# lRomul/sensorium

Measured on AMD Instinct MI355X. Metric: training clips/sec/GPU (DwiseNeuro fwd+bwd, B=32 T=32 36x64) at 1/2/4/8 GPUs, higher is better.
Workload: dtype bf16

## Files before the change

sensorium_amd/csrc/dwn_api.hip:

```cpp
#include "dwn_internal.h"
#include "dwn_kernels.h"
#include <string.h>
#include <math.h>

static thread_local char g_err[512] = "";
#ifndef DWN_EVAL_CHAIN
#define DWN_EVAL_CHAIN 1
#endif

extern "C" size_t dwn_dw_spatial_rc_blob_bytes(int E, int Cin);
extern "C" int dwn_dw_spatial_rc_supported(int dtype, int Cin, int E, int ks, int stride, int Hin, int Win);
extern "C" int dwn_dw_spatial_rc_prep(const float* w_pw, const float* w_dws, const float* bn1_coef, int E, int Cin, void* blob,
                                      int device, void* stream);
extern "C" int dwn_dw_spatial_fwd_rc(const dwn_dw_spatial_rc_fwd_args* a, int device, void* stream);
bool dw_spatial_bwd_rc_supported(const DwSpatialBwd& a, int dtype);
bool dw_spatial_fwd_rc_walk_supported(const DwSpatialFwd& a, int dtype);

int dwn_set_error(int code, const char* msg) {
    snprintf(g_err, sizeof(g_err), "dwn error %d: %s", code, msg ? msg : "");
    return code;
}

#define TRY(x) do { int rc__ = (x); if (rc__ != 0) return rc__; } while (0)

// ... 124 lines not shown
GemmTN tn_base(const LoadDesc& p, int pk, const LoadDesc& q, int qk, int M, int R, int Cc, float* dw, i64 lddw, int groups) {
    GemmTN g; memset(&g, 0, sizeof(g));
    g.p = p; g.p_kind = pk; g.q = q; g.q_kind = qk; g.M = M; g.R = R; g.Cc = Cc; g.dw = dw; g.lddw = lddw;
    g.groups = groups; g.nsplit = 0;
    return g;
}

struct BlockWs {
    void *wpw, *wpwl;
    float *wdws, *wdwt;
    double *st1, *st2, *st3, *st4, *stsc;
    long long* pooled;
    float *abc1, *abc2, *abc3, *abc4, *abcsc, *ident3;
    float *dgp, *dhp, *dps;
    void* bp; float* r3; float* gacc;
    float* tacc;
    void* wgated;
    void* rcblob;
    double* gram;
    float* pb;
    char* zero_beg; char* zero_end;
    size_t bytes;
};
#ifndef PWL_GATED_MIN_ROWS
#define PWL_GATED_MIN_ROWS 8192
#endif
static bool pwl_gated_weights(const dwn_block_args& a) {
    const int bk = a.dtype == DWN_BF16 ? 64 : 32;
    return ((a.T * a.Hout * a.Wout) % 128) == 0 && a.Cmid > bk && (a.dtype != DWN_BF16 || a.T * a.Hout * a.Wout >= PWL_GATED_MIN_ROWS);
}
// ... 44 lines not shown
    if (!backward && block_y1_free(a)) w.gram = c.take<double>((size_t)(a.Cin + 8) * a.Cin);
    size_t z1 = c.off;
    if (backward) {
        w.abc1 = c.take<float>(3 * (size_t)a.Cmid);
        w.abc2 = c.take<float>(3 * (size_t)a.Cmid);
        w.abc3 = c.take<float>(3 * (size_t)a.Cmid);
        w.abc4 = c.take<float>(3 * (size_t)a.Cout);
        w.abcsc = c.take<float>(3 * (size_t)a.Cout);
        w.ident3 = c.take<float>(3 * (size_t)a.Cmid);
        w.dgp = c.take<float>((size_t)a.B * a.Cmid);
        w.dhp = c.take<float>((size_t)a.B * a.se_r);
        w.dps = c.take<float>((size_t)a.B * a.Cmid);
        w.bp = c.take<char>((size_t)a.Cin * (a.Cmid + a.Cin) * ts);
        w.gacc = c.take<float>(pw_fold_floats(a.Cin));
        w.r3 = w.gacc + (size_t)a.Cin * a.Cin;
        w.tacc = c.take<float>(pw_wgrad_tacc_floats(a.Cmid, a.Cin));
        if (pwl_bwd_per_sample(a)) w.pb = c.take<float>((size_t)a.B * a.Cout * a.Cmid);
    }
    w.bytes = c.off + 256;
    if (base) { w.zero_beg = (char*)base + z0; w.zero_end = (char*)base + z1; }
    return w;
}

static inline int f32_split_of(int policy, bool eval_forward) {
    return policy == DWN_F32_SPLIT3 ? 1 : policy == DWN_F32_NATIVE ? 0 : (eval_forward ? 1 : 0);
}

ResGeom geom_of(const dwn_block_args& a) {
    ResGeom gm;
    gm.BT = a.B * a.T; gm.T = a.T; gm.Hin = a.Hin; gm.Win = a.Win; gm.Hout = a.Hout; gm.Wout = a.Wout;
// ... 343 lines not shown
        g.stats = tr ? w.st4 : nullptr; g.stat_nchan = a.Cout; g.f32_split = f32_split_of(a.f32_products, !tr);
        PROF(DWN_FAM_PWL_FWD, launch_gemm_nn(g, dt, s));
    }
    ResGeom gm = geom_of(a);
    if (bs) {
        if (!(y1_free && identity_sc)) PROF(DWN_FAM_RESID_FWD, k_shortcut_stats(xin, gm, w.stsc, dt, s));
        TRY(k_bn_finalize_train(fin_job(w.st4, a.Cout, (double)Mout, a.bn4, a.Cout),
                                 fin_job(w.stsc, a.Cin, (double)Mout, a.bnsc, a.Cout), a.momentum, a.eps, s));
    }
    PROF(DWN_FAM_RESID_FWD, k_residual_fwd(xin, a.y4, a.bn4.coef, a.bnsc.coef, a.drop_scale, gm, a.out_pe_t, a.out_pe_h,
                                           a.out_pe_w, a.out, dt, s));
    return 0;
}

static int pw_backward(int dt, const void* dh1, const void* a0, const float* w_pw, const float* abc, int E, int Cin, i64 M,
                       void* bp, float* gacc, float* r3, float* tacc, void* da0, float* dw, const void* res,
                       const float* res_abc, int res_C, const ResGeom* rg, hipStream_t s) {
    const int res_n = res ? res_C / Cin : 0;
    const bool gathered = res && rg && rg->hinv;
    if (res && (!res_abc || res_C % Cin || res_n < 1 || res_n > 2))
        return dwn_set_error(-2, "pw_backward: the shortcut term needs res_abc and res_C in {Cin, 2 Cin}");
    if (res && !pw_bwd_fused_supported(dt, M, E, Cin))
        return dwn_set_error(-3, "pw_backward: the shortcut term is built into the one-pass kernel only (dwn_pw_bwd_fused_supported)");
    TRY(k_pw_bwd_prep(w_pw, abc, E, Cin, bp, gacc, r3, dt, (res && !gathered) ? res_abc : nullptr, res_C, s));
    if (pw_bwd_fused_supported(dt, M, E, Cin)) {
        PROF(DWN_FAM_PW_DGRAD, launch_pw_bwd_fused(dh1, a0, bp, r3, da0, tacc, M, E, Cin, dt, res, res_abc, res_n,
                                                   gathered ? rg->hinv : nullptr, gathered ? rg->winv : nullptr, gathered ? rg->Hin : 0,
                                                   gathered ? rg->Win : 0, gathered ? rg->Hout : 0, gathered ? rg->Wout : 0, s));
    } else {
        {
            GemmNN g = nn_base(ld_plain(dh1, E), LD_PLAIN, bp, (i64)E + Cin, da0, Cin, (int)M, Cin, E + Cin, 1);
            g.epi = EPI_STORE_CAT; g.a2 = a0; g.a2_ld = Cin; g.K1 = E; g.bias = r3;
            PROF(DWN_FAM_PW_DGRAD, launch_gemm_nn(g, dt, s));
        }
        {
            LoadDesc cat = ld_plain(dh1, E);
            cat.q = a0; cat.ld2 = Cin; cat.cat_c1 = E; cat.cat_c2 = Cin;
            GemmTN g = tn_base(cat, LD_CAT1, ld_plain(a0, Cin), LD_PLAIN, (int)M, E + Cin + 8, Cin, tacc, Cin, 1);
            PROF(DWN_FAM_PW_WGRAD, launch_gemm_tn(g, dt, s));
// ... 19 lines not shown
    float* dg = reinterpret_cast<float*>(w.pooled);
    const bool y1_free = block_y1_free(a);
    {
        PrepArgs pa;
        bool ok = pa.zero(w.zero_beg, ((size_t)(w.zero_end - w.zero_beg) + 15) & ~(size_t)15);
        ok = ok && pa.packw(a.w_pwl, w.wpwl, 1, a.Cout, a.Cmid, 1, a.Cmid, a.Cout);
        if (y1_free) ok = ok && pa.packw(a.w_pw, w.wpw, 1, a.Cmid, a.Cin, 0, a.Cmid, a.Cin);
        ok = ok && pa.packdw(a.w_dws, w.wdws, a.Cmid, a.ks * a.ks);
        ok = ok && pa.packdw(a.w_dwt, w.wdwt, a.Cmid, a.kt);
        ok = ok && pa.fill(w.ident3, 1.0f, a.Cmid);
        ok = ok && pa.fill(w.ident3 + a.Cmid, 0.0f, 2 * a.Cmid);
        ok = ok && pa.zero(a.dw_dws, (size_t)a.Cmid * a.ks * a.ks * sizeof(float));
        ok = ok && pa.zero(a.dw_dwt, (size_t)a.Cmid * a.kt * sizeof(float));
        ok = ok && pa.zero(a.dw_pwl, (size_t)a.Cout * a.Cmid * sizeof(float));
        if (w.pb) ok = ok && pa.zero(w.pb, (size_t)a.B * a.Cout * a.Cmid * sizeof(float));
        ok = ok && pa.zero(w.gacc, pw_fold_floats(a.Cin) * sizeof(float));
        ok = ok && pa.zero(w.tacc, pw_wgrad_tacc_floats(a.Cmid, a.Cin) * sizeof(float));
        if (!ok) return dwn_set_error(-2, "block_backward: workspace arena and dw_* buffers must be 16-byte aligned");
        TRY(k_prep(pa, dt, s));
    }

    LoadDesc xin = ld_plain(a.x_has_pe ? a.x : a.a0, a.Cin);
    ResGeom gm = geom_of(a);
    PROF(DWN_FAM_RESID_BWD, k_residual_bwd_reduce(xin, a.y4, a.dout, a.bn4.coef, a.bnsc.coef, a.drop_scale, gm, w.st4, w.stsc, dt, s));
    TRY(k_bn_bwd_finalize(bwd_job(w.st4, (double)Mout, a.bn4, w.abc4, a.Cout, frozen),
                          bwd_job(w.stsc, (double)Mout, a.bnsc, w.abcsc, a.Cout, frozen), s));
    PROF(DWN_FAM_RESID_BWD, k_residual_bwd_dy4(a.y4, a.dout, w.abc4, a.drop_scale, gm, a.dy4, dt, s));
    void* du = a.buf_a;
    if (w.pb) {
        {
            GemmTN g = tn_base(ld_plain(a.dy4, a.Cout), LD_PLAIN, ld_plain(a.z3, a.Cmid), LD_PLAIN, (int)Mout, a.Cout,
// ... 43 lines not shown
    TRY(k_bn_bwd_finalize(bwd_job(w.st2, (double)Mout, a.bn2, w.abc2, a.Cmid, frozen), BnBwdJob{}, s));
    void* dh1 = a.buf_a;
    {
        DwSpatialBwd d; memset(&d, 0, sizeof(d));
        d.dy = ld_affine2(a.buf_b, a.y2, a.Cmid, w.abc2, a.Cmid);
        d.y1 = ld_ycoef(y1_free ? nullptr : a.y1, a.Cmid, a.bn1.coef, a.Cmid);
        if (y1_free) { d.a0 = xin.p; d.a0_ld = a.Cin; d.w1 = w.wpw; d.Cin = a.Cin; }
        d.w = w.wdws; d.dh1 = dh1; d.dw = a.dw_dws; d.planes = a.B * a.T; d.Hin = a.Hin; d.Win = a.Win;
        d.Hout = a.Hout; d.Wout = a.Wout; d.C = a.Cmid; d.stride = a.stride; d.ks = a.ks; d.stats = w.st1;
        PROF(DWN_FAM_DWS_BWD, launch_dw_spatial_bwd(d, dt, s));
    }
    TRY(k_bn_bwd_finalize(bwd_job(w.st1, (double)Min, a.bn1, w.abc1, a.Cmid, frozen), BnBwdJob{}, s));
    const bool identity_sc = a.stride == 1 && a.Hin == a.Hout && a.Win == a.Wout;
    const bool dx_folded = a.Cout % a.Cin == 0 && a.Cout / a.Cin <= 2 && dwn_pw_bwd_fused_supported(dt, Min, a.Cmid, a.Cin) &&
                           (identity_sc || (gm.hinv && gm.winv && a.Hin + a.Win <= 512));
    TRY(pw_backward(dt, dh1, xin.p, a.w_pw, w.abc1, a.Cmid, a.Cin, Min, w.bp, w.gacc, w.r3, w.tacc, dx_folded ? a.dx : a.da0, a.dw_pw,
                    dx_folded ? a.dout : nullptr, w.abcsc, a.Cout, (dx_folded && !identity_sc) ? &gm : nullptr, s));
    if (dx_folded) return 0;
    PROF(DWN_FAM_RESID_BWD, k_residual_bwd_dx(xin, a.da0, a.dout, w.abcsc, gm, a.dx, dt, s));
    return 0;
}

int dwn_block_forward_writes(const dwn_block_args* ap) {
    const dwn_block_args& a = *ap;
    if (a.training) return block_y1_free(a) ? 2 : 3;
    if (block_fwd_rc(a)) return 0;
    if (DWN_EVAL_CHAIN && a.dtype == DWN_BF16) {
        DwSpatialFwd f; memset(&f, 0, sizeof(f));
        f.planes = a.B * a.T; f.Hin = a.Hin; f.Win = a.Win; f.Hout = a.Hout; f.Wout = a.Wout; f.C = a.Cmid; f.stride = a.stride; f.ks = a.ks;
        f.in.ld = a.Cmid; f.a0_ld = a.Cin; f.Cin = a.Cin;
        if (dw_spatial_fwd_rc_walk_supported(f, a.dtype)) return 0;
// ... 258 lines not shown
    g_err[0] = 0;
    if (ntensors < 0) return dwn_set_error(-2, "adamw_ema_multi_guarded: ntensors < 0");
    if (max_blocks < 1 || max_blocks > 65535 || ntensors > 65535)
        return dwn_set_error(-2, "adamw_ema_multi_guarded: max_blocks and ntensors are grid dimensions (1 <= max_blocks, both <= 65535)");
    if (!list && ntensors > 0) return dwn_set_error(-1, "adamw_ema_multi_guarded: null table");
    if (!guard) return dwn_set_error(-1, "adamw_ema_multi_guarded: null guard");
    ENTER(device);
    return k_adamw_ema_guarded(list, ntensors, max_blocks, lr, beta1, beta2, eps, weight_decay, ema_decay, grad_scale, guard,
                               (hipStream_t)stream);
}

int dwn_pw_bwd_fused_supported(int dtype, long long M, int E, int Cin) {
    return pw_bwd_fused_supported(dtype, M, E, Cin) ? 1 : 0;
}
size_t dwn_pw_backward_workspace_bytes(int E, int Cin, int dtype) {
    return (size_t)Cin * (E + Cin) * tsize(dtype) + 256 + (pw_fold_floats(Cin) + pw_wgrad_tacc_floats(E, Cin)) * sizeof(float) + 256;
}
int dwn_pw_backward(const dwn_pw_bwd_args* a, int dtype, int device, void* stream) {
    ENTER(device);
    if (!a || !a->dh1 || !a->a0 || !a->w_pw || !a->abc || !a->da0 || !a->dw || !a->ws)
        return dwn_set_error(-1, "pw_backward: null pointer");
    if (a->E <= 0 || a->Cin <= 0 || a->E % 8 || a->Cin % 8 || a->M <= 0 || a->M > 0x7fffffffLL)
        return dwn_set_error(-2, "pw_backward: E and Cin must be positive multiples of 8, 0 < M < 2^31");
    if (a->ws_bytes < dwn_pw_backward_workspace_bytes(a->E, a->Cin, dtype)) return dwn_set_error(-6, "pw_backward: workspace too small");
    hipStream_t s = (hipStream_t)stream;
    Carver c(a->ws, a->ws_bytes);
    void* bp = c.take<char>((size_t)a->Cin * (a->E + a->Cin) * tsize(dtype));
    const size_t nz = pw_fold_floats(a->Cin) + pw_wgrad_tacc_floats(a->E, a->Cin);
    float* gacc = c.take<float>(nz);
    float* r3 = gacc + (size_t)a->Cin * a->Cin;
    float* tacc = gacc + pw_fold_floats(a->Cin);
    TRY(k_zero(gacc, nz * sizeof(float), s));
    ResGeom rg; memset(&rg, 0, sizeof(rg));
    rg.hinv = a->res_hinv; rg.winv = a->res_winv; rg.Hin = a->res_Hin; rg.Win = a->res_Win; rg.Hout = a->res_Hout; rg.Wout = a->res_Wout;
    return pw_backward(dtype, a->dh1, a->a0, a->w_pw, a->abc, a->E, a->Cin, a->M, bp, gacc, r3, tacc, a->da0, a->dw, a->res,
                       a->res_abc, a->res_C, a->res_hinv ? &rg : nullptr, s);
}

int dwn_assemble_inputs(const dwn_clip_desc* descs, int B, int T, int H0, int W0, int H, int W, float pad_fill,
                        float* x, int device, void* stream) {
    ENTER(device);
    if (!descs || !x) return dwn_set_error(-1, "assemble_inputs: null pointer");
    if (B <= 0 || T <= 0 || H0 <= 0 || W0 <= 0) return dwn_set_error(-2, "assemble_inputs: B, T, H0, W0 must be positive");
    if (H < H0 || W < W0) return dwn_set_error(-2, "assemble_inputs: output frame smaller than the video");
    return k_assemble_inputs(descs, B, T, H0, W0, H, W, pad_fill, x, (hipStream_t)stream);
}

int dwn_assemble_targets(const dwn_clip_desc* descs, int B, int T, float* const* targets, const int* n_neurons,
                         int n_mice, int max_neurons, float* mice_weights, int device, void* stream) {
    ENTER(device);
// ... 80 lines not shown
```

sensorium_amd/csrc/dwn_elementwise.hip:

```cpp
#include "dwn_internal.h"
#include "dwn_kernels.h"
#include "dwn_launch.h"

#define NCV 8
#define DISPATCH_T(dtype, CALL_BF, CALL_F) do { if ((dtype) == DWN_BF16) { CALL_BF; } else { CALL_F; } } while (0)

#define SLICE_SETUP(Cval)                                   \
    constexpr int KC = TT<T>::KC;                           \
    const int tid = threadIdx.x;                            \
    const int cv = tid % NCV, pl = tid / NCV;               \
    const int c0 = blockIdx.y * NCV * KC;                   \
    const int chan = c0 + cv * KC;                          \
    const bool chan_ok = chan < (Cval);                     \
    (void)pl; (void)chan_ok;

template <int KC>
__device__ __forceinline__ void slice_stats_flush(float* lstat, const float* s0, const float* s1, int cv,
                                                 int c0, int C, double* stats, int rep) {
    static_assert(NCV == 8, "wave pre-reduction below assumes 8 channel vectors per slice");
    const int tid = threadIdx.x;
    DET_WAVES_BEGIN
#pragma unroll
    for (int i = 0; i < KC; ++i) {
        float a = s0[i], b = s1[i];
// ... 1223 lines not shown
    const int c_end = (part + 1) * per < C ? (part + 1) * per : C;
    for (int c = part * per + tid; c < c_end; c += 256) {
        float acc = 0.f;
        for (int r = 0; r < R; ++r) acc = fmaf(wr[(i64)r * C + c], dhp[r], acc);
        dps[(i64)b * C + c] = acc * inv_s;
    }
}

#define SE_RT 64
__device__ __forceinline__ float wave_sum(float v) {
#pragma unroll
    for (int o = 32; o > 0; o >>= 1) v += __shfl_xor(v, o);
    return v;
}

template <int RP>
__global__ __launch_bounds__(256) void se_mlp_fwd_rows_kernel(const long long* pooled_sum, float inv_s, const float* wr,
                                                              const float* br, const float* we, const float* be, int C,
                                                              int R, float* pmean, float* hid_pre, float* gate,
                                                              const float* __restrict__ w2, void* __restrict__ wg, int N2, int wg_bf16) {
    constexpr int RPW = RP / 4;
    __shared__ float hid[RP];
    __shared__ float gl[256];
    const int b = blockIdx.x, tid = threadIdx.x, lane = tid & 63, wave = tid >> 6;
    const int split = gridDim.y, part = blockIdx.y;
    const int C4 = C >> 2;
    float acc[RPW];
#pragma unroll
    for (int q = 0; q < RPW; ++q) acc[q] = 0.f;
    const longlong2* ps2 = reinterpret_cast<const longlong2*>(pooled_sum + (i64)b * C);
    float4* pm4 = reinterpret_cast<float4*>(pmean + (i64)b * C);
    for (int c4 = lane; c4 < C4; c4 += 64) {
        const longlong2 p0 = ps2[2 * c4], p1 = ps2[2 * c4 + 1];
        float4 v;
        v.x = pool_unfix(p0.x) * inv_s; v.y = pool_unfix(p0.y) * inv_s; v.z = pool_unfix(p1.x) * inv_s; v.w = pool_unfix(p1.y) * inv_s;
        if (part == 0 && wave == 0) pm4[c4] = v;
        float4 w[RPW];
#pragma unroll
        for (int q = 0; q < RPW; ++q) {
            const int r = wave + 4 * q;
            w[q] = reinterpret_cast<const float4*>(wr + (i64)(r < R ? r : R - 1) * C)[c4];
        }
#pragma unroll
        for (int q = 0; q < RPW; ++q)
            acc[q] = fmaf(w[q].x, v.x, fmaf(w[q].y, v.y, fmaf(w[q].z, v.z, fmaf(w[q].w, v.w, acc[q]))));
    }
#pragma unroll
    for (int q = 0; q < RPW; ++q) {
        const float t = wave_sum(acc[q]);
        const int r = wave + 4 * q;
        if (lane == 0 && r < R) {
            const float h = t + br[r];
            if (part == 0) hid_pre[(i64)b * R + r] = h;
            hid[r] = siluf_(h);
        }
    }
    __syncthreads();
    const int per = (C + split - 1) / split;
    const int c_end = (part + 1) * per < C ? (part + 1) * per : C;
    for (int c = part * per + tid; c < c_end; c += 256) {
        float a = be[c];
        const float* wrow = we + (i64)c * R;
#pragma unroll 1
        for (int r0 = 0; r0 < RP; r0 += 16) {
            if (r0 >= R) break;
            float wv[16];
            if ((R & 3) == 0) {
                const float4* w4 = reinterpret_cast<const float4*>(wrow);
                const int nq = R >> 2;
#pragma unroll
                for (int q = 0; q < 4; ++q) {
                    const int qi = (r0 >> 2) + q;
                    const float4 t = w4[qi < nq ? qi : nq - 1];
                    wv[4 * q] = t.x; wv[4 * q + 1] = t.y; wv[4 * q + 2] = t.z; wv[4 * q + 3] = t.w;
                }
            } else {
#pragma unroll
                for (int r = 0; r < 16; ++r) wv[r] = wrow[r0 + r < R ? r0 + r : R - 1];
            }
#pragma unroll
            for (int r = 0; r < 16; ++r) a = fmaf(wv[r], r0 + r < R ? hid[r0 + r] : 0.f, a);
        }
        const float gv = sigmoidf_(a);
        gate[(i64)b * C + c] = gv;
        if (w2 && c - part * per < 256) gl[c - part * per] = gv;
    }
    if (w2) {
        __syncthreads();
        const int c0 = part * per, nc = c_end - c0;
        if (nc > 0) {
            const int tot = N2 * nc;
            for (int i = tid; i < tot; i += 256) {
                const int n = i / nc, cc = i - n * nc;
                const float v = w2[(i64)n * C + c0 + cc] * gl[cc];
                const i64 o = ((i64)b * N2 + n) * C + c0 + cc;
                if (wg_bf16) reinterpret_cast<bf16_t*>(wg)[o] = f2bf(v);
                else reinterpret_cast<float*>(wg)[o] = v;
            }
        }
    }
}

template <int N, int LIVE, int D> struct WaveFold {
    static __device__ __forceinline__ void run(float (&v)[N], int lane) {
        if constexpr (D > 0) {
            if constexpr (LIVE > D) {
                constexpr int H = LIVE / 2;
// ... 81 lines not shown
            float wv[16];
#pragma unroll
            for (int r = 0; r < 16; ++r) wv[r] = wr[(i64)(r0 + r < R ? r0 + r : R - 1) * C + c];
#pragma unroll
            for (int r = 0; r < 16; ++r) a = fmaf(wv[r], r0 + r < R ? dhp[r0 + r] : 0.f, a);
        }
        dps[(i64)b * C + c] = a * inv_s;
    }
}

__global__ __launch_bounds__(256) void se_mlp_wgrad_kernel(const float* dgp, const float* dhp, const float* pmean,
                                                           const float* hid_pre, int B, int C, int R, float* dwr,
                                                           float* dbr, float* dwe, float* dbe) {
    const int c = blockIdx.x * 256 + threadIdx.x;
    const int r = blockIdx.y;
    if (c < C) {
        float a = 0.f, a2 = 0.f, sb = 0.f;
#pragma unroll 8
        for (int b = 0; b < B; ++b) {
            float g = dgp[(i64)b * C + c];
            a = fmaf(g, siluf_(hid_pre[(i64)b * R + r]), a);
            a2 = fmaf(dhp[(i64)b * R + r], pmean[(i64)b * C + c], a2);
            sb += g;
        }
        dwe[(i64)c * R + r] = a;
        dwr[(i64)r * C + c] = a2;
        if (r == 0) dbe[c] = sb;
    }
    if (blockIdx.x == 0 && threadIdx.x == 0) {
        float sb = 0.f;
        for (int b = 0; b < B; ++b) sb += dhp[(i64)b * R + r];
        dbr[r] = sb;
    }
}

int k_se_mlp_fwd(const long long* pooled_sum, float inv_s, const float* wr, const float* br, const float* we,
                 const float* be, int B, int C, int R, float* pmean, float* hid_pre, float* gate, const float* w2, void* wg, int N2,
                 int dtype, int* folded, hipStream_t s) {
    if (folded) *folded = 0;
    if ((C & 3) == 0 && R <= SE_RT && !(((size_t)pooled_sum | (size_t)wr | (size_t)pmean) & 15)) {
        const bool fold = w2 && wg && (C + 7) / 8 <= 256;
        const float* w2f = fold ? w2 : nullptr;
        const int bf = dtype == DWN_BF16 ? 1 : 0;
        if (R <= 16)
            hipLaunchKernelGGL(se_mlp_fwd_rows_kernel<16>, dim3(B, 8), dim3(256), 0, s, pooled_sum, inv_s, wr, br, we, be, C, R,
                               pmean, hid_pre, gate, w2f, wg, N2, bf);
        else if (R <= 32)
            hipLaunchKernelGGL(se_mlp_fwd_rows_kernel<32>, dim3(B, 8), dim3(256), 0, s, pooled_sum, inv_s, wr, br, we, be, C, R,
                               pmean, hid_pre, gate, w2f, wg, N2, bf);
        else
            hipLaunchKernelGGL(se_mlp_fwd_rows_kernel<SE_RT>, dim3(B, 8), dim3(256), 0, s, pooled_sum, inv_s, wr, br, we, be, C,
                               R, pmean, hid_pre, gate, w2f, wg, N2, bf);
        if (folded && fold) *folded = 1;
    } else {
        hipLaunchKernelGGL(se_mlp_fwd_kernel, dim3(B, 8), dim3(256), (C + R) * sizeof(float), s, pooled_sum, inv_s, wr, br,
                           we, be, C, R, pmean, hid_pre, gate);
    }
    DWN_CHECK_LAUNCH();
    return 0;
}
int k_se_mlp_bwd(const float* dg, const float* gate, const float* hid_pre, const float* pmean, const float* wr,
                 const float* we, int B, int C, int R, float inv_s, float* dgp, float* dhp, float* dps, float* dwr,
                 float* dbr, float* dwe, float* dbe, hipStream_t s) {
    if ((R & 1) == 0 && R <= SE_RT && !((size_t)we & 15)) {
#define SE_BWD_FOLD(RP_) do { \
        if ((R & 3) == 0) hipLaunchKernelGGL((se_mlp_bwd_fold_kernel<RP_, 4>), dim3(B, 8), dim3(256), 0, s, dg, gate, hid_pre, wr, we, C, R, inv_s, dgp, dhp, dps); \
        else hipLaunchKernelGGL((se_mlp_bwd_fold_kernel<RP_, 2>), dim3(B, 8), dim3(256), 0, s, dg, gate, hid_pre, wr, we, C, R, inv_s, dgp, dhp, dps); } while (0)
// ... 990 lines not shown
int k_prep(const PrepArgs& pa, int dtype, hipStream_t s) {
    int total = 0;
    for (int i = 0; i < pa.nops; ++i) total += pa.op[i].nblocks;
    if (total == 0) return 0;
    DISPATCH_T(dtype,
        hipLaunchKernelGGL((prep_kernel<bf16_t>), dim3(total), dim3(256), 0, s, pa),
        hipLaunchKernelGGL((prep_kernel<float>), dim3(total), dim3(256), 0, s, pa));
    DWN_CHECK_LAUNCH();
    return 0;
}



template <typename T>
__global__ __launch_bounds__(256) void pw_bwd_prep_kernel(const float* w1, const float* abc, int E, int C, T* bp, float* gacc,
                                                          float* r3, int nscale, int gx, int gy, int gr) {
    const i64 ld = (i64)E + C;
    int bid = blockIdx.x;
    __shared__ float sA[64][64 + 4], sB[64][64 + 4];
    if (bid < nscale) {
        const int nkt = (E + 63) / 64;
        const int k0 = (bid % nkt) * 64, n0 = (bid / nkt) * 64;
        for (int i = threadIdx.x; i < 64 * 64; i += 256) {
            const int kl = i >> 6, nl = i & 63;
            const int k = k0 + kl, n = n0 + nl;
            sA[kl][nl] = (k < E && n < C) ? abc[k] * round_t<T>(w1[(i64)k * C + n]) : 0.f;
        }
        __syncthreads();
        for (int i = threadIdx.x; i < 64 * 64; i += 256) {
            const int nl = i >> 6, kl = i & 63;
            const int k = k0 + kl, n = n0 + nl;
// ... 29 lines not shown
#pragma unroll 8
    for (int el = 0; el < GR; ++el) {
        const float4 a4 = *reinterpret_cast<const float4*>(&sA[el][ty * 4]);
        const float4 b4 = *reinterpret_cast<const float4*>(&sB[el][tx * 4]);
        const float a[4] = {a4.x, a4.y, a4.z, a4.w}, b[4] = {b4.x, b4.y, b4.z, b4.w};
#pragma unroll
        for (int i = 0; i < 4; ++i)
#pragma unroll
            for (int j = 0; j < 4; ++j) acc[i][j] = fmaf(a[i], b[j], acc[i][j]);
        if (do_r3) {
            const float a3 = e0 + el < E ? A3[e0 + el] : 0.f;
#pragma unroll
            for (int j = 0; j < 4; ++j) acc3[j] = fmaf(a3, b[j], acc3[j]);
        }
    }
    DET_ENTER();
#pragma unroll
    for (int i = 0; i < 4; ++i) {
        const int cp = bx * 64 + ty * 4 + i;
#pragma unroll
        for (int j = 0; j < 4; ++j) {
            const int c = by * 64 + tx * 4 + j;
            if (cp < C && c < C) atomicAdd(gacc + (i64)cp * C + c, acc[i][j]);
        }
    }
    if (do_r3) {
#pragma unroll
        for (int j = 0; j < 4; ++j) {
            const int c = by * 64 + tx * 4 + j;
            if (c < C) atomicAdd(r3 + c, acc3[j]);
        }
    }
    DET_EXIT();
}
template <typename T>
__global__ __launch_bounds__(256) void pw_bwd_gram_store_kernel(const float* gacc, int E, int C, T* bp, const float* res_abc, int res_C,
                                                                float* r3) {
    const i64 idx = (i64)blockIdx.x * 256 + threadIdx.x;
    if (idx >= (i64)C * C) return;
    const int cp = (int)(idx / C), c = (int)(idx % C);
    float g = gacc[idx];
    if (res_abc && cp == c) {
        float d2 = 0.f, d3 = 0.f;
        for (int cc = c; cc < res_C; cc += C) { d2 += res_abc[res_C + cc]; d3 += res_abc[2 * res_C + cc]; }
        g += d2;
        r3[c] += d3;
    }
    bp[(i64)c * ((i64)E + C) + E + cp] = from_f<T>(g);
}
int k_pw_bwd_prep(const float* w1, const float* abc, int E, int C, void* bp, float* gacc, float* r3, int dtype,
                  const float* res_abc, int res_C, hipStream_t s) {
    const int nscale = ((E + 63) / 64) * ((C + 63) / 64);
    const int gr = C <= 64 ? 32 : 64;
    const int gx = (C + 63) / 64, gy = (C + 63) / 64, gz = (E + gr - 1) / gr;
    const int ngram = gx * gy * gz;
    DISPATCH_T(dtype,
        hipLaunchKernelGGL((pw_bwd_prep_kernel<bf16_t>), dim3(nscale + ngram), dim3(256), 0, s, w1, abc, E, C, (bf16_t*)bp, gacc, r3, nscale, gx, gy, gr),
        hipLaunchKernelGGL((pw_bwd_prep_kernel<float>), dim3(nscale + ngram), dim3(256), 0, s, w1, abc, E, C, (float*)bp, gacc, r3, nscale, gx, gy, gr));
    DWN_CHECK_LAUNCH();
    dim3 g3((unsigned)(((i64)C * C + 255) / 256));
    DISPATCH_T(dtype,
        hipLaunchKernelGGL((pw_bwd_gram_store_kernel<bf16_t>), g3, dim3(256), 0, s, gacc, E, C, (bf16_t*)bp, res_abc, res_C, r3),
        hipLaunchKernelGGL((pw_bwd_gram_store_kernel<float>), g3, dim3(256), 0, s, gacc, E, C, (float*)bp, res_abc, res_C, r3));
    DWN_CHECK_LAUNCH();
    return 0;
}

size_t pw_wgrad_tacc_floats(int E, int C) { return (size_t)(E + C + 8) * C; }
template <typename T>
__global__ __launch_bounds__(256) void pw_wgrad_fold_kernel(const float* __restrict__ tacc, const float* __restrict__ abc,
                                                            const float* __restrict__ w1, int E, int C, float* __restrict__ dw) {
    const i64 idx = (i64)blockIdx.x * 256 + threadIdx.x;
    if (idx >= (i64)E * C) return;
    const int e = (int)(idx / C), c = (int)(idx % C);
    const float* ga = tacc + (i64)E * C + c;
    const float* wrow = w1 + (i64)e * C;
    float g0 = 0.f, g1 = 0.f, g2 = 0.f, g3 = 0.f;
    for (int cp = 0; cp < C; cp += 4) {
// ... 63 lines not shown
```

sensorium_amd/csrc/dwn_kernels.h:

```cpp
#pragma once
#include "dwn_internal.h"

struct ResGeom {
    int BT, T, Hin, Win, Hout, Wout, Cin, Cout;
    const int* hsrc; const int* wsrc;
    const int* hinv; const int* winv;
};

typedef dwn_tensor_entry TensorListEntry;

struct BnFinJob {
    const double* stats; int stat_c; double count; const float* gamma; const float* beta;
    float* running_mean; float* running_var; long long* nbt; float* coef; int C; int nblocks;
};
struct BnBwdJob { const double* stats; double count; const float* coef; float* dgamma; float* dbeta; float* abc; int C; int nblocks; int frozen; };
int k_bn_finalize_train(BnFinJob j0, BnFinJob j1, float momentum, float eps, hipStream_t s);
int k_bn_bwd_finalize(BnBwdJob j0, BnBwdJob j1, hipStream_t s);
int k_bn_finalize_eval(const float* gamma, const float* beta, const float* rm, const float* rv, float eps,
                       float* coef, int C, hipStream_t s);
int k_bn1_gram_finalize(const double* gram, const float* w1, int E, int Cin, double count, const float* gamma, const float* beta,
                        float* rm, float* rv, long long* nbt, float momentum, float eps, float* coef, double* sc_stats, int dtype,
                        hipStream_t s);
int k_ew_apply(const LoadDesc& d, int kind, void* out, i64 ldo, i64 rows, int C, int dtype, hipStream_t s);
int k_stem_xmom(const float* x, int B, int Cin, i64 S, double* mom, hipStream_t s);
// ... 75 lines not shown
                       hipStream_t s);
int k_pwl_bwd_reduce(const float* P, const float* gate, const float* W, int B, int K, int N, float* dW, float* dg,
                     hipStream_t s);
int k_assemble_inputs(const dwn_clip_desc* descs, int B, int T, int H0, int W0, int H, int W, float pad, float* x,
                      hipStream_t s);
int k_assemble_targets(const dwn_clip_desc* descs, int B, int T, float* const* targets, const int* n_neurons,
                       int n_mice, int max_neurons, float* mice_weights, hipStream_t s);
int k_zero(void* p, size_t nbytes, hipStream_t s);
int k_gaze_forward(const dwn_gaze_args& a, hipStream_t s);
int k_gaze_backward(const dwn_gaze_args& a, hipStream_t s);
int k_plane_mean(const float* x, int B, int Cin, int T, int H, int W, int c0, int nc, float* mean, hipStream_t s);
size_t k_corr_ws_bytes(int N);
int k_corr_moments(const dwn_corr_args& a, hipStream_t s);
int k_corr_finalize(const dwn_corr_args& a, hipStream_t s);
int k_corr_backward(const dwn_corr_args& a, hipStream_t s);
int k_pw_bwd_prep(const float* w1, const float* abc, int E, int C, void* bp, float* gacc, float* r3, int dtype,
                  const float* res_abc, int res_C, hipStream_t s);
size_t pw_wgrad_tacc_floats(int E, int C);
int k_pw_wgrad_fold(const float* tacc, const float* abc, const float* w1, int E, int C, float* dw, int dtype, hipStream_t s);

enum { PREP_ZERO = 0, PREP_FILL = 1, PREP_PACKW = 2, PREP_PACKDW = 3, PREP_BNEVAL = 4 };
#define PREP_MAX_OPS 16
struct PrepOp {
    int kind, nblocks;
    const float* src; void* dst;
    const float* src2; const float* src3; const float* src4;
    long long n;
    float v;
    int R, C, transpose, Rd, Cd;
};
struct PrepArgs {
// ... 37 lines not shown
```

Before: 1472.

## Use gram slabs in pw backward prep and rework SE MLP fwd/bwd kernels

When Cin is at least 128, the pointwise-backward prep kernel writes per-chunk gram partials into a slab buffer instead of accumulating atomically into gacc. The gram store kernel then sums the slabs, and the gacc zeroing is skipped in that case. Separately, the SE MLP forward rows kernel moves to 1024 threads with pooled means staged in LDS and weights prefetched in registers. The SE MLP weight-gradient kernel is re-indexed so dwe is written coalesced, with batched loads. The price is extra workspace, higher register pressure, and a serial slab reduction.

```diff
diff --git a/sensorium_amd/csrc/dwn_api.hip b/sensorium_amd/csrc/dwn_api.hip
--- a/sensorium_amd/csrc/dwn_api.hip
+++ b/sensorium_amd/csrc/dwn_api.hip
@@ -162,6 +162,7 @@
     float *abc1, *abc2, *abc3, *abc4, *abcsc, *ident3;
     float *dgp, *dhp, *dps;
     void* bp; float* r3; float* gacc;
+    float* gslab;
     float* tacc;
     void* wgated;
     void* rcblob;
@@ -236,6 +237,7 @@
         w.bp = c.take<char>((size_t)a.Cin * (a.Cmid + a.Cin) * ts);
         w.gacc = c.take<float>(pw_fold_floats(a.Cin));
         w.r3 = w.gacc + (size_t)a.Cin * a.Cin;
+        if (pw_gram_slab_floats(a.Cmid, a.Cin)) w.gslab = c.take<float>(pw_gram_slab_floats(a.Cmid, a.Cin));
         w.tacc = c.take<float>(pw_wgrad_tacc_floats(a.Cmid, a.Cin));
         if (pwl_bwd_per_sample(a)) w.pb = c.take<float>((size_t)a.B * a.Cout * a.Cmid);
     }
@@ -609,7 +611,7 @@
 }
 
 static int pw_backward(int dt, const void* dh1, const void* a0, const float* w_pw, const float* abc, int E, int Cin, i64 M,
-                       void* bp, float* gacc, float* r3, float* tacc, void* da0, float* dw, const void* res,
+                       void* bp, float* gacc, float* r3, float* gslab, float* tacc, void* da0, float* dw, const void* res,
                        const float* res_abc, int res_C, const ResGeom* rg, hipStream_t s) {
     const int res_n = res ? res_C / Cin : 0;
     const bool gathered = res && rg && rg->hinv;
@@ -617,7 +619,7 @@
         return dwn_set_error(-2, "pw_backward: the shortcut term needs res_abc and res_C in {Cin, 2 Cin}");
     if (res && !pw_bwd_fused_supported(dt, M, E, Cin))
         return dwn_set_error(-3, "pw_backward: the shortcut term is built into the one-pass kernel only (dwn_pw_bwd_fused_supported)");
-    TRY(k_pw_bwd_prep(w_pw, abc, E, Cin, bp, gacc, r3, dt, (res && !gathered) ? res_abc : nullptr, res_C, s));
+    TRY(k_pw_bwd_prep(w_pw, abc, E, Cin, bp, gacc, r3, gslab, dt, (res && !gathered) ? res_abc : nullptr, res_C, s));
     if (pw_bwd_fused_supported(dt, M, E, Cin)) {
         PROF(DWN_FAM_PW_DGRAD, launch_pw_bwd_fused(dh1, a0, bp, r3, da0, tacc, M, E, Cin, dt, res, res_abc, res_n,
                                                    gathered ? rg->hinv : nullptr, gathered ? rg->winv : nullptr, gathered ? rg->Hin : 0,
@@ -667,7 +669,7 @@
         ok = ok && pa.zero(a.dw_dwt, (size_t)a.Cmid * a.kt * sizeof(float));
         ok = ok && pa.zero(a.dw_pwl, (size_t)a.Cout * a.Cmid * sizeof(float));
         if (w.pb) ok = ok && pa.zero(w.pb, (size_t)a.B * a.Cout * a.Cmid * sizeof(float));
-        ok = ok && pa.zero(w.gacc, pw_fold_floats(a.Cin) * sizeof(float));
+        if (!w.gslab) ok = ok && pa.zero(w.gacc, pw_fold_floats(a.Cin) * sizeof(float));
         ok = ok && pa.zero(w.tacc, pw_wgrad_tacc_floats(a.Cmid, a.Cin) * sizeof(float));
         if (!ok) return dwn_set_error(-2, "block_backward: workspace arena and dw_* buffers must be 16-byte aligned");
         TRY(k_prep(pa, dt, s));
@@ -741,7 +743,7 @@
     const bool identity_sc = a.stride == 1 && a.Hin == a.Hout && a.Win == a.Wout;
     const bool dx_folded = a.Cout % a.Cin == 0 && a.Cout / a.Cin <= 2 && dwn_pw_bwd_fused_supported(dt, Min, a.Cmid, a.Cin) &&
                            (identity_sc || (gm.hinv && gm.winv && a.Hin + a.Win <= 512));
-    TRY(pw_backward(dt, dh1, xin.p, a.w_pw, w.abc1, a.Cmid, a.Cin, Min, w.bp, w.gacc, w.r3, w.tacc, dx_folded ? a.dx : a.da0, a.dw_pw,
+    TRY(pw_backward(dt, dh1, xin.p, a.w_pw, w.abc1, a.Cmid, a.Cin, Min, w.bp, w.gacc, w.r3, w.gslab, w.tacc, dx_folded ? a.dx : a.da0, a.dw_pw,
                     dx_folded ? a.dout : nullptr, w.abcsc, a.Cout, (dx_folded && !identity_sc) ? &gm : nullptr, s));
     if (dx_folded) return 0;
     PROF(DWN_FAM_RESID_BWD, k_residual_bwd_dx(xin, a.da0, a.dout, w.abcsc, gm, a.dx, dt, s));
@@ -1030,7 +1032,8 @@
     return pw_bwd_fused_supported(dtype, M, E, Cin) ? 1 : 0;
 }
 size_t dwn_pw_backward_workspace_bytes(int E, int Cin, int dtype) {
-    return (size_t)Cin * (E + Cin) * tsize(dtype) + 256 + (pw_fold_floats(Cin) + pw_wgrad_tacc_floats(E, Cin)) * sizeof(float) + 256;
+    return (size_t)Cin * (E + Cin) * tsize(dtype) + 256 + (pw_fold_floats(Cin) + pw_wgrad_tacc_floats(E, Cin)) * sizeof(float) + 256 +
+           pw_gram_slab_floats(E, Cin) * sizeof(float) + 256;
 }
 int dwn_pw_backward(const dwn_pw_bwd_args* a, int dtype, int device, void* stream) {
     ENTER(device);
@@ -1046,10 +1049,11 @@
     float* gacc = c.take<float>(nz);
     float* r3 = gacc + (size_t)a->Cin * a->Cin;
     float* tacc = gacc + pw_fold_floats(a->Cin);
+    float* gslab = pw_gram_slab_floats(a->E, a->Cin) ? c.take<float>(pw_gram_slab_floats(a->E, a->Cin)) : nullptr;
     TRY(k_zero(gacc, nz * sizeof(float), s));
     ResGeom rg; memset(&rg, 0, sizeof(rg));
     rg.hinv = a->res_hinv; rg.winv = a->res_winv; rg.Hin = a->res_Hin; rg.Win = a->res_Win; rg.Hout = a->res_Hout; rg.Wout = a->res_Wout;
-    return pw_backward(dtype, a->dh1, a->a0, a->w_pw, a->abc, a->E, a->Cin, a->M, bp, gacc, r3, tacc, a->da0, a->dw, a->res,
+    return pw_backward(dtype, a->dh1, a->a0, a->w_pw, a->abc, a->E, a->Cin, a->M, bp, gacc, r3, gslab, tacc, a->da0, a->dw, a->res,
                        a->res_abc, a->res_C, a->res_hinv ? &rg : nullptr, s);
 }
 
diff --git a/sensorium_amd/csrc/dwn_elementwise.hip b/sensorium_amd/csrc/dwn_elementwise.hip
--- a/sensorium_amd/csrc/dwn_elementwise.hip
+++ b/sensorium_amd/csrc/dwn_elementwise.hip
@@ -1261,83 +1261,122 @@
     return v;
 }
 
+#define SE_NT 1024
+static inline size_t se_fwd_rows_lds(int C, int RP) { return ((size_t)C + RP + 256) * sizeof(float); }
 template <int RP>
-__global__ __launch_bounds__(256) void se_mlp_fwd_rows_kernel(const long long* pooled_sum, float inv_s, const float* wr,
-                                                              const float* br, const float* we, const float* be, int C,
-                                                              int R, float* pmean, float* hid_pre, float* gate,
-                                                              const float* __restrict__ w2, void* __restrict__ wg, int N2, int wg_bf16) {
-    constexpr int RPW = RP / 4;
-    __shared__ float hid[RP];
-    __shared__ float gl[256];
+__global__ __launch_bounds__(SE_NT) void se_mlp_fwd_rows_kernel(const long long* pooled_sum, float inv_s, const float* wr,
+                                                                const float* br, const float* we, const float* be, int C,
+                                                                int R, float* pmean, float* hid_pre, float* gate,
+                                                                const float* __restrict__ w2, void* __restrict__ wg, int N2, int wg_bf16) {
+    constexpr int NW = SE_NT / 64, RPW = RP / NW, NS = RP <= 16 ? 2 : 4;
+    extern __shared__ __attribute__((aligned(16))) float se_lds[];
+    float* pm = se_lds;
+    float* hid = se_lds + C;
+    float* gl = hid + RP;
     const int b = blockIdx.x, tid = threadIdx.x, lane = tid & 63, wave = tid >> 6;
     const int split = gridDim.y, part = blockIdx.y;
     const int C4 = C >> 2;
+    const int nsteps = (C4 + 63) >> 6;
+    const float4* wrow4[RPW];
+    float brv[RPW];
+#pragma unroll
+    for (int q = 0; q < RPW; ++q) {
+        const int r = wave + NW * q;
+        wrow4[q] = reinterpret_cast<const float4*>(wr + (i64)(r < R ? r : R - 1) * C);
+    }
+    float4 w[NS][RPW];
+    auto load_round = [&](int s0) {
+#pragma unroll
+        for (int j = 0; j < NS; ++j) {
+            const int c4 = lane + 64 * (s0 + j);
+#pragma unroll
+            for (int q = 0; q < RPW; ++q) w[j][q] = wrow4[q][c4 < C4 ? c4 : C4 - 1];
+        }
+    };
+    load_round(0);
+#pragma unroll
+    for (int q = 0; q < RPW; ++q) brv[q] = br[wave + NW * q < R ? wave + NW * q : R - 1];
+    {
+        const longlong2* ps2 = reinterpret_cast<const longlong2*>(pooled_sum + (i64)b * C);
+        float2* pm2 = reinterpret_cast<float2*>(pmean + (i64)b * C);
+        for (int i = tid; i < (C >> 1); i += SE_NT) {
+            const longlong2 p = ps2[i];
+            float2 v;
+            v.x = pool_unfix(p.x) * inv_s; v.y = pool_unfix(p.y) * inv_s;
+            reinterpret_cast<float2*>(pm)[i] = v;
+            if (part == 0) pm2[i] = v;
+        }
+    }
+    __syncthreads();
     float acc[RPW];
 #pragma unroll
     for (int q = 0; q < RPW; ++q) acc[q] = 0.f;
-    const longlong2* ps2 = reinterpret_cast<const longlong2*>(pooled_sum + (i64)b * C);
-    float4* pm4 = reinterpret_cast<float4*>(pmean + (i64)b * C);
-    for (int c4 = lane; c4 < C4; c4 += 64) {
-        const longlong2 p0 = ps2[2 * c4], p1 = ps2[2 * c4 + 1];
-        float4 v;
-        v.x = pool_unfix(p0.x) * inv_s; v.y = pool_unfix(p0.y) * inv_s; v.z = pool_unfix(p1.x) * inv_s; v.w = pool_unfix(p1.y) * inv_s;
-        if (part == 0 && wave == 0) pm4[c4] = v;
-        float4 w[RPW];
-#pragma unroll
-        for (int q = 0; q < RPW; ++q) {
-            const int r = wave + 4 * q;
-            w[q] = reinterpret_cast<const float4*>(wr + (i64)(r < R ? r : R - 1) * C)[c4];
-        }
-#pragma unroll
-        for (int q = 0; q < RPW; ++q)
-            acc[q] = fmaf(w[q].x, v.x, fmaf(w[q].y, v.y, fmaf(w[q].z, v.z, fmaf(w[q].w, v.w, acc[q]))));
+    for (int s0 = 0;;) {
+#pragma unroll
+        for (int j = 0; j < NS; ++j) {
+            const int c4 = lane + 64 * (s0 + j);
+            float4 v = reinterpret_cast<const float4*>(pm)[c4 < C4 ? c4 : C4 - 1];
+            if (c4 >= C4) v = make_float4(0.f, 0.f, 0.f, 0.f);
+#pragma unroll
+            for (int q = 0; q < RPW; ++q)
+                acc[q] = fmaf(w[j][q].x, v.x, fmaf(w[j][q].y, v.y, fmaf(w[j][q].z, v.z, fmaf(w[j][q].w, v.w, acc[q]))));
+        }
+        s0 += NS;
+        if (s0 >= nsteps) break;
+        load_round(s0);
     }
 #pragma unroll
     for (int q = 0; q < RPW; ++q) {
         const float t = wave_sum(acc[q]);
-        const int r = wave + 4 * q;
+        const int r = wave + NW * q;
         if (lane == 0 && r < R) {
-            const float h = t + br[r];
+            const float h = t + brv[q];
             if (part == 0) hid_pre[(i64)b * R + r] = h;
             hid[r] = siluf_(h);
         }
     }
-    __syncthreads();
     const int per = (C + split - 1) / split;
     const int c_end = (part + 1) * per < C ? (part + 1) * per : C;
-    for (int c = part * per + tid; c < c_end; c += 256) {
-        float a = be[c];
-        const float* wrow = we + (i64)c * R;
-#pragma unroll 1
-        for (int r0 = 0; r0 < RP; r0 += 16) {
-            if (r0 >= R) break;
-            float wv[16];
-            if ((R & 3) == 0) {
-                const float4* w4 = reinterpret_cast<const float4*>(wrow);
-                const int nq = R >> 2;
-#pragma unroll
-                for (int q = 0; q < 4; ++q) {
-                    const int qi = (r0 >> 2) + q;
-                    const float4 t = w4[qi < nq ? qi : nq - 1];
-                    wv[4 * q] = t.x; wv[4 * q + 1] = t.y; wv[4 * q + 2] = t.z; wv[4 * q + 3] = t.w;
-                }
-            } else {
-#pragma unroll
-                for (int r = 0; r < 16; ++r) wv[r] = wrow[r0 + r < R ? r0 + r : R - 1];
-            }
-#pragma unroll
-            for (int r = 0; r < 16; ++r) a = fmaf(wv[r], r0 + r < R ? hid[r0 + r] : 0.f, a);
-        }
+    __builtin_amdgcn_sched_barrier(0);
+    const int c = part * per + tid;
+    const bool act = c < c_end;
+    float a, wv[RP];
+    {
+        const int cl = act ? c : c_end - 1;
+        a = be[cl];
+        const float* wrow = we + (i64)cl * R;
+        if ((R & 3) == 0) {
+            const float4* w4 = reinterpret_cast<const float4*>(wrow);
+            const int nq = R >> 2;
+#pragma unroll
+            for (int q = 0; q < RP / 4; ++q) {
+                const float4 t = w4[q < nq ? q : nq - 1];
+                wv[4 * q] = t.x; wv[4 * q + 1] = t.y; wv[4 * q + 2] = t.z; wv[4 * q + 3] = t.w;
+            }
+        } else {
+#pragma unroll
+            for (int r = 0; r < RP; ++r) {
+                wv[r] = wrow[r < R ? r : R - 1];
+                if ((r & 15) == 15) __builtin_amdgcn_sched_barrier(0);
+            }
+        }
+    }
+    __syncthreads();
+    if (act) {
+#pragma unroll
+        for (int r = 0; r < RP; ++r)
+            if (r < R) a = fmaf(wv[r], hid[r], a);
         const float gv = sigmoidf_(a);
         gate[(i64)b * C + c] = gv;
-        if (w2 && c - part * per < 256) gl[c - part * per] = gv;
+        if (w2 && tid < 256) gl[tid] = gv;
     }
     if (w2) {
         __syncthreads();
         const int c0 = part * per, nc = c_end - c0;
         if (nc > 0) {
             const int tot = N2 * nc;
-            for (int i = tid; i < tot; i += 256) {
+#pragma unroll 4
+            for (int i = tid; i < tot; i += SE_NT) {
                 const int n = i / nc, cc = i - n * nc;
                 const float v = w2[(i64)n * C + c0 + cc] * gl[cc];
                 const i64 o = ((i64)b * N2 + n) * C + c0 + cc;
@@ -1449,23 +1488,37 @@
                                                            float* dbr, float* dwe, float* dbe) {
     const int c = blockIdx.x * 256 + threadIdx.x;
     const int r = blockIdx.y;
+    constexpr int NB = 32;
+    const i64 e = ((i64)blockIdx.y * gridDim.x + blockIdx.x) * 256 + threadIdx.x;
+    const bool eok = e < (i64)C * R;
+    const int ce = eok ? (int)(e / R) : 0, re = eok ? (int)(e % R) : 0;
+    const int cc = c < C ? c : C - 1;
+    float a = 0.f, a2 = 0.f, sb = 0.f, sd = 0.f;
+    for (int b0 = 0; b0 < B; b0 += NB) {
+        float g[NB], p[NB], h[NB], d[NB], ge[NB];
+#pragma unroll
+        for (int j = 0; j < NB; ++j) {
+            const int b = b0 + j < B ? b0 + j : B - 1;
+            g[j] = dgp[(i64)b * C + cc];
+            p[j] = pmean[(i64)b * C + cc];
+            d[j] = dhp[(i64)b * R + r];
+            ge[j] = dgp[(i64)b * C + ce];
+            h[j] = hid_pre[(i64)b * R + re];
+        }
+#pragma unroll
+        for (int j = 0; j < NB; ++j)
+            if (b0 + j < B) {
+                a = fmaf(ge[j], siluf_(h[j]), a);
+                a2 = fmaf(d[j], p[j], a2);
+                sb += g[j];
+                sd += d[j];
+            }
+    }
+    if (eok) dwe[e] = a;
     if (c < C) {
-        float a = 0.f, a2 = 0.f, sb = 0.f;
-#pragma unroll 8
-        for (int b = 0; b < B; ++b) {
-            float g = dgp[(i64)b * C + c];
-            a = fmaf(g, siluf_(hid_pre[(i64)b * R + r]), a);
-            a2 = fmaf(dhp[(i64)b * R + r], pmean[(i64)b * C + c], a2);
-            sb += g;
-        }
-        dwe[(i64)c * R + r] = a;
         dwr[(i64)r * C + c] = a2;
         if (r == 0) dbe[c] = sb;
-    }
-    if (blockIdx.x == 0 && threadIdx.x == 0) {
-        float sb = 0.f;
-        for (int b = 0; b < B; ++b) sb += dhp[(i64)b * R + r];
-        dbr[r] = sb;
+        if (c == 0) dbr[r] = sd;
     }
 }
 
@@ -1473,19 +1526,19 @@
                  const float* be, int B, int C, int R, float* pmean, float* hid_pre, float* gate, const float* w2, void* wg, int N2,
                  int dtype, int* folded, hipStream_t s) {
     if (folded) *folded = 0;
-    if ((C & 3) == 0 && R <= SE_RT && !(((size_t)pooled_sum | (size_t)wr | (size_t)pmean) & 15)) {
+    if ((C & 3) == 0 && C <= 8 * SE_NT && R <= SE_RT && !(((size_t)pooled_sum | (size_t)wr | (size_t)pmean) & 15)) {
         const bool fold = w2 && wg && (C + 7) / 8 <= 256;
         const float* w2f = fold ? w2 : nullptr;
         const int bf = dtype == DWN_BF16 ? 1 : 0;
         if (R <= 16)
-            hipLaunchKernelGGL(se_mlp_fwd_rows_kernel<16>, dim3(B, 8), dim3(256), 0, s, pooled_sum, inv_s, wr, br, we, be, C, R,
-                               pmean, hid_pre, gate, w2f, wg, N2, bf);
+            hipLaunchKernelGGL(se_mlp_fwd_rows_kernel<16>, dim3(B, 8), dim3(SE_NT), se_fwd_rows_lds(C, 16), s, pooled_sum, inv_s, wr, br,
+                               we, be, C, R, pmean, hid_pre, gate, w2f, wg, N2, bf);
         else if (R <= 32)
-            hipLaunchKernelGGL(se_mlp_fwd_rows_kernel<32>, dim3(B, 8), dim3(256), 0, s, pooled_sum, inv_s, wr, br, we, be, C, R,
-                               pmean, hid_pre, gate, w2f, wg, N2, bf);
+            hipLaunchKernelGGL(se_mlp_fwd_rows_kernel<32>, dim3(B, 8), dim3(SE_NT), se_fwd_rows_lds(C, 32), s, pooled_sum, inv_s, wr, br,
+                               we, be, C, R, pmean, hid_pre, gate, w2f, wg, N2, bf);
         else
-            hipLaunchKernelGGL(se_mlp_fwd_rows_kernel<SE_RT>, dim3(B, 8), dim3(256), 0, s, pooled_sum, inv_s, wr, br, we, be, C,
-                               R, pmean, hid_pre, gate, w2f, wg, N2, bf);
+            hipLaunchKernelGGL(se_mlp_fwd_rows_kernel<SE_RT>, dim3(B, 8), dim3(SE_NT), se_fwd_rows_lds(C, SE_RT), s, pooled_sum, inv_s, wr,
+                               br, we, be, C, R, pmean, hid_pre, gate, w2f, wg, N2, bf);
         if (folded && fold) *folded = 1;
     } else {
         hipLaunchKernelGGL(se_mlp_fwd_kernel, dim3(B, 8), dim3(256), (C + R) * sizeof(float), s, pooled_sum, inv_s, wr, br,
@@ -2506,7 +2559,7 @@
 
 template <typename T>
 __global__ __launch_bounds__(256) void pw_bwd_prep_kernel(const float* w1, const float* abc, int E, int C, T* bp, float* gacc,
-                                                          float* r3, int nscale, int gx, int gy, int gr) {
+                                                          float* r3, float* gslab, int nscale, int gx, int gy, int gr) {
     const i64 ld = (i64)E + C;
     int bid = blockIdx.x;
     __shared__ float sA[64][64 + 4], sB[64][64 + 4];
@@ -2566,6 +2619,28 @@
             for (int j = 0; j < 4; ++j) acc3[j] = fmaf(a3, b[j], acc3[j]);
         }
     }
+    if (gslab) {
+        float* gs = gslab + (i64)bz * ((i64)C * C + C);
+#pragma unroll
+        for (int i = 0; i < 4; ++i) {
+            const int cp = bx * 64 + ty * 4 + i, c = by * 64 + tx * 4;
+            if (cp < C && c + 3 < C && (C & 3) == 0)
+                *reinterpret_cast<float4*>(gs + (i64)cp * C + c) = make_float4(acc[i][0], acc[i][1], acc[i][2], acc[i][3]);
+            else
+#pragma unroll
+                for (int j = 0; j < 4; ++j)
+                    if (cp < C && c + j < C) gs[(i64)cp * C + c + j] = acc[i][j];
+        }
+        if (do_r3) {
+#pragma unroll
+            for (int j = 0; j < 4; ++j) {
+                const int c = by * 64 + tx * 4 + j;
+                if (c < C) gs[(i64)C * C + c] = acc3[j];
+            }
+        }
+        DET_EXIT();
+        return;
+    }
     DET_ENTER();
 #pragma unroll
     for (int i = 0; i < 4; ++i) {
@@ -2587,33 +2662,55 @@
 }
 template <typename T>
 __global__ __launch_bounds__(256) void pw_bwd_gram_store_kernel(const float* gacc, int E, int C, T* bp, const float* res_abc, int res_C,
-                                                                float* r3) {
+                                                                float* r3, const float* __restrict__ gslab, int nslab) {
     const i64 idx = (i64)blockIdx.x * 256 + threadIdx.x;
     if (idx >= (i64)C * C) return;
     const int cp = (int)(idx / C), c = (int)(idx % C);
-    float g = gacc[idx];
+    float g = 0.f, r = 0.f;
+    if (gslab) {
+        const i64 ss = (i64)C * C + C;
+        constexpr int SU = 16;
+        for (int z0 = 0; z0 < nslab; z0 += SU) {
+            float v[SU], v3[SU];
+#pragma unroll
+            for (int u = 0; u < SU; ++u) {
+                const int z = z0 + u < nslab ? z0 + u : nslab - 1;
+                v[u] = gslab[z * ss + idx];
+                v3[u] = cp == c ? gslab[z * ss + (i64)C * C + c] : 0.f;
+            }
+#pragma unroll
+            for (int u = 0; u < SU; ++u)
+                if (z0 + u < nslab) { g += v[u]; r += v3[u]; }
+        }
+    } else {
+        g = gacc[idx];
+        if (cp == c) r = r3[c];
+    }
     if (res_abc && cp == c) {
         float d2 = 0.f, d3 = 0.f;
         for (int cc = c; cc < res_C; cc += C) { d2 += res_abc[res_C + cc]; d3 += res_abc[2 * res_C + cc]; }
         g += d2;
-        r3[c] += d3;
-    }
+        r += d3;
+    }
+    if (cp == c && (gslab || res_abc)) r3[c] = r;
     bp[(i64)c * ((i64)E + C) + E + cp] = from_f<T>(g);
 }
-int k_pw_bwd_prep(const float* w1, const float* abc, int E, int C, void* bp, float* gacc, float* r3, int dtype,
+size_t pw_gram_slab_floats(int E, int C) { return C >= 128 ? (size_t)((E + 63) / 64) * ((size_t)C * C + C) : 0; }
+int k_pw_bwd_prep(const float* w1, const float* abc, int E, int C, void* bp, float* gacc, float* r3, float* gslab, int dtype,
                   const float* res_abc, int res_C, hipStream_t s) {
     const int nscale = ((E + 63) / 64) * ((C + 63) / 64);
     const int gr = C <= 64 ? 32 : 64;
     const int gx = (C + 63) / 64, gy = (C + 63) / 64, gz = (E + gr - 1) / gr;
     const int ngram = gx * gy * gz;
+    if (pw_gram_slab_floats(E, C) == 0) gslab = nullptr;
     DISPATCH_T(dtype,
-        hipLaunchKernelGGL((pw_bwd_prep_kernel<bf16_t>), dim3(nscale + ngram), dim3(256), 0, s, w1, abc, E, C, (bf16_t*)bp, gacc, r3, nscale, gx, gy, gr),
-        hipLaunchKernelGGL((pw_bwd_prep_kernel<float>), dim3(nscale + ngram), dim3(256), 0, s, w1, abc, E, C, (float*)bp, gacc, r3, nscale, gx, gy, gr));
+        hipLaunchKernelGGL((pw_bwd_prep_kernel<bf16_t>), dim3(nscale + ngram), dim3(256), 0, s, w1, abc, E, C, (bf16_t*)bp, gacc, r3, gslab, nscale, gx, gy, gr),
+        hipLaunchKernelGGL((pw_bwd_prep_kernel<float>), dim3(nscale + ngram), dim3(256), 0, s, w1, abc, E, C, (float*)bp, gacc, r3, gslab, nscale, gx, gy, gr));
     DWN_CHECK_LAUNCH();
     dim3 g3((unsigned)(((i64)C * C + 255) / 256));
     DISPATCH_T(dtype,
-        hipLaunchKernelGGL((pw_bwd_gram_store_kernel<bf16_t>), g3, dim3(256), 0, s, gacc, E, C, (bf16_t*)bp, res_abc, res_C, r3),
-        hipLaunchKernelGGL((pw_bwd_gram_store_kernel<float>), g3, dim3(256), 0, s, gacc, E, C, (float*)bp, res_abc, res_C, r3));
+        hipLaunchKernelGGL((pw_bwd_gram_store_kernel<bf16_t>), g3, dim3(256), 0, s, gacc, E, C, (bf16_t*)bp, res_abc, res_C, r3, gslab, gz),
+        hipLaunchKernelGGL((pw_bwd_gram_store_kernel<float>), g3, dim3(256), 0, s, gacc, E, C, (float*)bp, res_abc, res_C, r3, gslab, gz));
     DWN_CHECK_LAUNCH();
     return 0;
 }
diff --git a/sensorium_amd/csrc/dwn_kernels.h b/sensorium_amd/csrc/dwn_kernels.h
--- a/sensorium_amd/csrc/dwn_kernels.h
+++ b/sensorium_amd/csrc/dwn_kernels.h
@@ -113,7 +113,8 @@
 int k_corr_moments(const dwn_corr_args& a, hipStream_t s);
 int k_corr_finalize(const dwn_corr_args& a, hipStream_t s);
 int k_corr_backward(const dwn_corr_args& a, hipStream_t s);
-int k_pw_bwd_prep(const float* w1, const float* abc, int E, int C, void* bp, float* gacc, float* r3, int dtype,
+size_t pw_gram_slab_floats(int E, int C);
+int k_pw_bwd_prep(const float* w1, const float* abc, int E, int C, void* bp, float* gacc, float* r3, float* gslab, int dtype,
                   const float* res_abc, int res_C, hipStream_t s);
 size_t pw_wgrad_tacc_floats(int E, int C);
 int k_pw_wgrad_fold(const float* tacc, const float* abc, const float* w1, int E, int C, float* dw, int dtype, hipStream_t s);
```

New measurement: 1482, median of 6. About the same (+0.7%).
